# dmalyuta/explicit_hybrid_mpc

Hardware: AMD Instinct MI355X
Metric: oracle LP solves/sec + final regions/sec, 4-state 2-input N=5 hybrid MPC (higher is better)
Workload: dtype f64

## Files before the change

explicit_hybrid_mpc_amd/csrc/ehm_ipm2.h:

```cpp
#include "ehm_dev.h"

#ifndef EHM_NP
#error "EHM_NP (column capacity, multiple of 4) must be defined"
#endif
#ifndef EHM_SLOTS
#error "EHM_SLOTS (row slots per lane) must be defined"
#endif

#ifndef EHM2_UNROLL
#define EHM2_UNROLL 2
#endif
#ifndef EHM2_FORM_MFMA
#define EHM2_FORM_MFMA 0
#endif
#ifndef EHM2_LU_CHUNK
#define EHM2_LU_CHUNK 8
#endif
#define EHM2_TOL_RES      1e-10
#define EHM2_TOL_GAP      1e-10
#define EHM2_MAX_ITER     40
#define EHM2_STEP_FRAC    0.999
#define EHM2_STEP_FRAC_SAFE 0.99
#define EHM2_STEP_FRAC_LAST 0.9
#define EHM2_ATTEMPTS     3
#define EHM2_PIVOT_REL    1e-13
#define EHM2_PIVOT_BIG    1e128
#define EHM2_STALL_ZONE   1e4
#define EHM2_ACCEPT_MERIT 1e3

#define EHM2_CAT2(a, b, c) a##b##_##c
#define EHM2_CAT(a, b, c) EHM2_CAT2(a, b, c)
#ifndef EHM2_QUAD
#define EHM2_QUAD 0
#endif
#if EHM2_QUAD
#define EHM2_NS EHM2_CAT(ehm2q_, EHM_NP, EHM_SLOTS)
#else
#define EHM2_NS EHM2_CAT(ehm2_, EHM_NP, EHM_SLOTS)
#endif

#ifndef EHM2_PROF
#define EHM2_PROF 0
#endif

namespace EHM2_NS {

using namespace ehm;

#if EHM2_PROF
#define EHM2_PT(k)                                                                   \
    {                                                                                \
        const long long _t = (long long)__builtin_readcyclecounter();               \
        if (lane0 == 0) W.pf[k] += (unsigned long long)(_t - _tp);                   \
        _tp = _t;                                                                    \
    }
#define EHM2_PDUMP()                                                                 \
    {                                                                                \
        wsync();                                                                     \
        if (S.gprof && lane0 < 24)                                                   \
            atomicAdd(&S.gprof[lane0], W.pf[lane0] + (lane0 == 23 ? 1ULL : 0ULL));   \
    }
#elif defined(EHM2_ISA_MARKS)
#define EHM2_PT(k) asm volatile("; @@PHASE " #k);
#define EHM2_PDUMP()
#else
#define EHM2_PT(k)
#define EHM2_PDUMP()
#endif

constexpr int NP = EHM_NP;
constexpr int SLOTS = EHM_SLOTS;
constexpr int MROWS = 64 * SLOTS;

__device__ __forceinline__ void wsync() {
    __builtin_amdgcn_fence(__ATOMIC_ACQ_REL, "wavefront");
    __builtin_amdgcn_wave_barrier();
}

template <int CTRL, int ROW_MASK>
__device__ __forceinline__ double dpp_move(double identity, double v) {
    const int lo = __builtin_amdgcn_update_dpp(__double2loint(identity), __double2loint(v), CTRL,
                                               ROW_MASK, 0xf, false);
    const int hi = __builtin_amdgcn_update_dpp(__double2hiint(identity), __double2hiint(v), CTRL,
                                               ROW_MASK, 0xf, false);
    return __hiloint2double(hi, lo);
}
__device__ __forceinline__ double lane63(double v) {
    const int lo = __builtin_amdgcn_readlane(__double2loint(v), 63);
    const int hi = __builtin_amdgcn_readlane(__double2hiint(v), 63);
    return __hiloint2double(hi, lo);
}
#define EHM2_DPP_REDUCE(OP, IDENT)                                       \
    v = OP(v, dpp_move<0x111, 0xf>(IDENT, v));                           \
    v = OP(v, dpp_move<0x112, 0xf>(IDENT, v));                           \
    v = OP(v, dpp_move<0x114, 0xf>(IDENT, v));                           \
    v = OP(v, dpp_move<0x118, 0xf>(IDENT, v));                           \
    v = OP(v, dpp_move<0x142, 0xa>(IDENT, v));                           \
    v = OP(v, dpp_move<0x143, 0xc>(IDENT, v));                           \
    return lane63(v);
__device__ __forceinline__ double op_add(double a, double b) { return a + b; }
__device__ __forceinline__ double op_max(double a, double b) { return fmax(a, b); }
__device__ __forceinline__ double op_min(double a, double b) { return fmin(a, b); }
#ifdef EHM2_REDUCE_SHFL
__device__ __forceinline__ double wave_sum(double v) {
    for (int o = 32; o > 0; o >>= 1) v += __shfl_xor(v, o, 64);
    return v;
}
__device__ __forceinline__ double wave_max(double v) {
    for (int o = 32; o > 0; o >>= 1) v = fmax(v, __shfl_xor(v, o, 64));
    return v;
}
#else
__device__ __forceinline__ double wave_sum(double v) { EHM2_DPP_REDUCE(op_add, 0.0) }
__device__ __forceinline__ double wave_max(double v) {
    EHM2_DPP_REDUCE(op_max, -__builtin_huge_val())
}
#endif
__device__ __forceinline__ double readlane_d(double v, int src) {
    const int lo = __builtin_amdgcn_readlane(__double2loint(v), src);
    const int hi = __builtin_amdgcn_readlane(__double2hiint(v), src);
    return __hiloint2double(hi, lo);
}
__device__ __forceinline__ int pin(int x) {
    asm volatile("" : "+v"(x));
    return x;
}
typedef __attribute__((address_space(3))) const volatile double lds_cvdouble;
__device__ __forceinline__ double lds1(const double* p) {
    return *(lds_cvdouble*)p;
}
__device__ __forceinline__ double uniform_d(double v) {
    int lo, hi;
    asm("s_nop 0\n\tv_readfirstlane_b32 %0, %2\n\tv_readfirstlane_b32 %1, %3\n\ts_nop 1"
        : "=s"(lo), "=s"(hi)
        : "v"(__double2loint(v)), "v"(__double2hiint(v)));
    return __hiloint2double(hi, lo);
}
__device__ __forceinline__ double const_d(double literal) {
    int lo = __double2loint(literal), hi = __double2hiint(literal);
    asm volatile("" : "+s"(lo), "+s"(hi));
    return __hiloint2double(hi, lo);
}
__device__ __forceinline__ double frcp(double x) {
    double r = __builtin_amdgcn_rcp(x);
    double e = fma(-x, r, 1.0);
    r = fma(r, e, r);
    e = fma(-x, r, 1.0);
    r = fma(r, e, r);
    return r;
}

struct Shared {
    const double* Wc;
    const double* wv;
    const double* cv;
    const double* aE;
    const double* eval;
    const int* erow;
    const int* eidx;
    int n, m, p, lda;
    int nd0, nE, LE;
    int colS, colOne, colZero;
#if EHM2_PROF
    unsigned long long* gprof;
#endif
};
__host__ __device__ inline size_t shared_doubles(const DevProblem& P) {
    return (((size_t)P.tot4 + (P.wc_lds ? P.m + P.n : 0)) + 1) & ~(size_t)1;
}
__device__ inline void carve_shared(Shared& S, double* base, const DevProblem& P) {
    S.n = P.n; S.m = P.m; S.p = P.p; S.lda = P.lda4;
    S.nd0 = P.nd0; S.nE = P.n - P.nd0; S.LE = P.LE4;
    S.colS = P.nd0; S.colOne = P.nd0 + P.p; S.colZero = P.nd0 + P.p + 1;
#if EHM2_PROF
    S.gprof = nullptr;
#endif
    S.Wc = base;
    S.aE = base + (size_t)(P.nd0 + P.p + 2) * P.lda4;
    S.eval = base + (size_t)P.ncw4 * P.lda4;
    S.erow = reinterpret_cast<const int*>(S.eval + (size_t)S.nE * S.LE);
    S.eidx = S.erow + (size_t)S.nE * S.LE;
    if (P.wc_lds) {
        S.wv = base + P.tot4;
        S.cv = S.wv + P.m;
    } else {
        S.wv = P.w;
        S.cv = P.c;
    }
}
__device__ inline void use_commutation(Shared& S, const DevProblem& P, int d) {
    if (!P.wc_lds) S.wv = P.w + (size_t)d * P.m;
}
__device__ inline void load_shared(const DevProblem& P, int d, double* base, int tid, int nthr) {
    const int tot = P.tot4;
    const double* src = P.Wc4 + (size_t)d * tot;
    for (int k = tid; k < tot; k += nthr) base[k] = src[k];
    if (P.wc_lds) {
        const double* wd = P.w + (size_t)d * P.m;
        for (int k = tid; k < P.m; k += nthr) base[tot + k] = wd[k];
        for (int k = tid; k < P.n; k += nthr) base[tot + P.m + k] = P.c[k];
    }
}

struct Wave {
    double* M;
    double* X;
    double* vm0;
    double* vm1;
    double* c;
    double* x;
    double* xb;
    double* t;
// ... 151 lines not shown
    int lane;
};
__device__ __forceinline__ void make_rowmap(RowMap& rm, const Shared& S, const Wave& W, int lane) {
    rm.lane = lane;
    const int zero_off = S.colZero * S.lda;
#pragma unroll
    for (int sl = 0; sl < SLOTS - 1; ++sl) rm.valid[sl] = (lane + 64 * sl) < S.m;
    const int i = lane + 64 * (SLOTS - 1);
    const bool spec = W.n_lin < W.nr;
    rm.last_extra = false;
    rm.last_sx = -1;
    if (i < S.m) {
        rm.valid[SLOTS - 1] = true;
        rm.last_base = S.Wc + i;
        rm.last_stride = S.lda;
        rm.last_spec = S.Wc + (spec ? W.spec_col * S.lda : zero_off) + i;
    } else if (i >= W.xbase + W.nsx && i < W.xbase + W.ne) {
        rm.valid[SLOTS - 1] = true;
        rm.last_extra = true;
        rm.last_base = W.X + (i - W.xbase - W.nsx);
        rm.last_stride = W.ldx;
        rm.last_spec = W.X + (size_t)W.n_lin * W.ldx + (i - W.xbase - W.nsx);
    } else if (i >= W.xbase && i < W.xbase + W.nsx) {
        rm.valid[SLOTS - 1] = true;
        rm.last_sx = i - W.xbase;
        rm.last_base = S.Wc + zero_off;
        rm.last_stride = 0;
        rm.last_spec = S.Wc + zero_off;
    } else {
        rm.valid[SLOTS - 1] = false;
        rm.last_base = S.Wc + zero_off;
        rm.last_stride = 0;
        rm.last_spec = S.Wc + zero_off;
    }
}

__device__ __forceinline__ void to_psi(const Wave& W, const double* v, int lane) {
    if (lane < NP) {
        double y = (lane < W.nr) ? v[lane] : 0.0;
        const int r = lane - W.psi0;
        if (r >= 0 && r < W.npsi) {
            y = 0.0;
            for (int q = 0; q < W.npsi; ++q) y = fma(W.E[r * W.npsi + q], v[W.psi0 + q], y);
        }
        W.yv[lane] = y;
    }
    wsync();
}

__device__ __forceinline__ void rows_times(const Shared& S, const Wave& W, int lane,
                                           const double* v, double (&out)[SLOTS]) {
    RowMap rm;
    make_rowmap(rm, S, W, lane);
    to_psi(W, v, rm.lane);
    const double* y = W.yv;
#pragma unroll
    for (int sl = 0; sl < SLOTS; ++sl) out[sl] = 0.0;
    const double* pa = S.Wc + rm.lane;
    const double* pb = rm.last_base;
    const double* pv = rm.last_extra ? v : y;
    const int lda = S.lda;
    const int str = rm.last_stride;
    int j = 0;
    constexpr int UR = EHM2_UNROLL;
    for (; j + UR - 1 < W.n_lin; j += UR) {
        double a[UR][SLOTS], yj[UR], vl[UR];
#pragma unroll
        for (int u = 0; u < UR; ++u) {
            yj[u] = y[j + u];
            vl[u] = lds1(pv + j + u);
#pragma unroll
            for (int sl = 0; sl < SLOTS - 1; ++sl) a[u][sl] = lds1(pa + u * lda + 64 * sl);
            a[u][SLOTS - 1] = lds1(pb + u * str);
        }
#pragma unroll
        for (int u = 0; u < UR; ++u) {
#pragma unroll
            for (int sl = 0; sl < SLOTS - 1; ++sl) out[sl] = fma(a[u][sl], yj[u], out[sl]);
            out[SLOTS - 1] = fma(a[u][SLOTS - 1], vl[u], out[SLOTS - 1]);
        }
        pa += UR * lda;
        pb += UR * str;
    }
    for (; j < W.n_lin; ++j) {
        const double yj = y[j];
#pragma unroll
        for (int sl = 0; sl < SLOTS - 1; ++sl) out[sl] = fma(lds1(pa + 64 * sl), yj, out[sl]);
        out[SLOTS - 1] = fma(lds1(pb), lds1(pv + j), out[SLOTS - 1]);
        pa += lda;
        pb += str;
    }
    if (W.n_lin < W.nr) {
        const double vj = v[W.n_lin];
        const double* ps = S.Wc + (size_t)W.spec_col * lda + rm.lane;
#pragma unroll
        for (int sl = 0; sl < SLOTS - 1; ++sl) out[sl] = fma(ps[64 * sl], vj, out[sl]);
        out[SLOTS - 1] = fma(*rm.last_spec, vj, out[SLOTS - 1]);
    }
    if (W.nE > 0) {
        const double* vE = v + W.nr;
#pragma unroll
        for (int sl = 0; sl < SLOTS; ++sl) {
            const int i = rm.lane + 64 * sl;
            const int ic = (i < S.m) ? i : 0;
            const double a = (i < S.m) ? S.aE[ic] : 0.0;
            out[sl] = fma(a, vE[S.eidx[ic]], out[sl]);
        }
        if (rm.last_extra) {
            const int xe = rm.lane + 64 * (SLOTS - 1) - W.xbase - W.nsx;
            const double* xr = W.X + (size_t)W.nr * W.ldx + xe;
            double a = 0.0;
            for (int e = 0; e < W.nE; ++e) a = fma(xr[(size_t)e * W.ldx], vE[e], a);
            out[SLOTS - 1] += a;
        }
    }
    if (W.nsx > 0) {
        double sb = 0.0;
        for (int q = 0; q < W.npsi; ++q) sb += v[W.psi0 + q];
        if (rm.last_sx >= 0)
            out[SLOTS - 1] = (rm.last_sx < W.npsi) ? -v[W.psi0 + (rm.last_sx < W.npsi ? rm.last_sx : 0)]
                                                  : sb;
    }
#pragma unroll
    for (int sl = 0; sl < SLOTS; ++sl) out[sl] = rm.valid[sl] ? out[sl] : 0.0;
}

__device__ __forceinline__ void block_cols_mpc(const Shared& S, const Wave& W, int cb,
                                               const double* (&pc)[4]) {
    const double* zero = S.Wc + (size_t)S.colZero * S.lda;
#pragma unroll
    for (int q = 0; q < 4; ++q) {
        const int j = 4 * cb + q;
        pc[q] = (j < W.nr) ? (S.Wc + (size_t)wc_col(W, j) * S.lda) : zero;
    }
}
__device__ __forceinline__ void block_cols_ext(const Shared& S, const Wave& W, int cb,
                                               const double* (&px)[4]) {
    const double* zero = S.Wc + (size_t)S.colZero * S.lda;
#pragma unroll
    for (int q = 0; q < 4; ++q) {
        const int j = 4 * cb + q;
        px[q] = (j < W.nr && W.ldx > 0) ? (W.X + (size_t)j * W.ldx) : zero;
    }
}

template <bool TWO>
__device__ __forceinline__ void cols_times(const Shared& S, const Wave& W, const double* u0,
                                           const double* u1, double* sc, int lane, double& r0,
                                           double& r1) {
    constexpr int nb = NP / 4;
    constexpr int ks = 64 / nb;
    double ex0 = 0.0, ex1 = 0.0;
    if (lane < W.n_lp && W.ne > W.nsx) {
        const double* xl = W.X + (size_t)lane * W.ldx;
        const int xb0 = W.xbase + W.nsx;
        for (int e = 0; e < W.ne - W.nsx; ++e) {
            const double a = xl[e];
            ex0 = fma(a, u0[xb0 + e], ex0);
            if (TWO) ex1 = fma(a, u1[xb0 + e], ex1);
        }
    }
    {
        const int q = lane - W.psi0;
        if (W.nsx > 0 && q >= 0 && q < W.npsi) {
            ex0 += u0[W.xbase + W.npsi] - u0[W.xbase + q];
            if (TWO) ex1 += u1[W.xbase + W.npsi] - u1[W.xbase + q];
        }
    }
    const int ecol = lane - W.nr;
    const bool elane = W.nE > 0 && ecol >= 0 && ecol < W.nE;
    if (W.nE > 0) {
        const int eb = (elane ? ecol : 0) * S.LE;
        double s0 = 0.0, s1 = 0.0;
        for (int k = 0; k < S.LE; k += 4) {
            int i[4];
            double a[4], w0[4], w1[4];
#pragma unroll
            for (int u = 0; u < 4; ++u) {
                i[u] = S.erow[eb + k + u];
                a[u] = S.eval[eb + k + u];
            }
#pragma unroll
            for (int u = 0; u < 4; ++u) {
                w0[u] = lds1(u0 + i[u]);
                w1[u] = TWO ? lds1(u1 + i[u]) : 0.0;
            }
#pragma unroll
            for (int u = 0; u < 4; ++u) {
                s0 = fma(a[u], w0[u], s0);
                if (TWO) s1 = fma(a[u], w1[u], s1);
            }
        }
        ex0 = elane ? (ex0 + s0) : ex0;
        if (TWO) ex1 = elane ? (ex1 + s1) : ex1;
    }
    const int cb = pin(lane % nb);
    const int h = pin(lane / nb);
    const bool active = h < ks;
    double a0[4] = {0.0, 0.0, 0.0, 0.0}, a1[4] = {0.0, 0.0, 0.0, 0.0};
    if (active) {
        const double* pc[4];
// ... 239 lines not shown
        }
    }
    if (m4 < m) {
        const bool in = m4 + lk < m;
        const int ic = in ? m4 : (m - 1 - lk);
        const double d = in ? lds1(pd + ic) : 0.0;
        const double w0 = lds1(p0 + ic);
        const double a0 = w0 * d;
        c00 = __builtin_amdgcn_mfma_f64_16x16x4f64(a0, w0, c00, 0, 0, 0);
        if (two) {
            const double w1 = lds1(p1 + ic);
            const double a1 = w1 * d;
            c10 = __builtin_amdgcn_mfma_f64_16x16x4f64(a1, w0, c10, 0, 0, 0);
            c11 = __builtin_amdgcn_mfma_f64_16x16x4f64(a1, w1, c11, 0, 0, 0);
        }
    }
    for (int e0 = 0; e0 < W.nE; e0 += 4) {
        const int e = e0 + lk;
        const bool in = e < W.nE;
        const int ec = in ? e : 0;
        const double id = W.iD[ec];
        const double g0 = (in && j0 < NP) ? W.gE[ec * GS + (j0 < NP ? j0 : 0)] : 0.0;
        c00 = __builtin_amdgcn_mfma_f64_16x16x4f64(-g0 * id, g0, c00, 0, 0, 0);
        if (two) {
            const double g1 = (in && j1 < NP) ? W.gE[ec * GS + (j1 < NP ? j1 : 0)] : 0.0;
            c10 = __builtin_amdgcn_mfma_f64_16x16x4f64(-g1 * id, g0, c10, 0, 0, 0);
            c11 = __builtin_amdgcn_mfma_f64_16x16x4f64(-g1 * id, g1, c11, 0, 0, 0);
        }
    }
    wsync();
#pragma unroll
    for (int r = 0; r < 4; ++r) {
        const int row = lk + 4 * r, col = li;
        if (row < NP && col < NP) W.M[row * LDM + col] = c00[r];
        if (two) {
            if (16 + row < NP && col < NP) {
                W.M[(16 + row) * LDM + col] = c10[r];
                W.M[col * LDM + 16 + row] = c10[r];
            }
            if (16 + row < NP && 16 + col < NP) W.M[(16 + row) * LDM + 16 + col] = c11[r];
        }
    }
}

__device__ __forceinline__ void form_eliminated(const Shared& S, const Wave& W, const double* dvec,
                                                int lane) {
    constexpr int NPG = (NP > 16) ? 32 : 16;
    const double* zero = S.Wc + (size_t)S.colZero * S.lda;
    const int ntask = W.nE * NPG;
    for (int t0 = 0; t0 < ntask; t0 += 64) {
        const int t = t0 + lane;
        const int r = t & (NPG - 1);
        const int e = t / NPG;
        const bool in = t < ntask;
        const double* col = (in && r < W.n_mpc) ? (S.Wc + (size_t)wc_col(W, r) * S.lda) : zero;
        const int eb = (in ? e : 0) * S.LE;
        double g = 0.0, dl = 0.0;
        for (int k = 0; k < S.LE; k += 4) {
            int i[4];
            double ev[4], dv[4], av[4];
#pragma unroll
            for (int u = 0; u < 4; ++u) {
                i[u] = S.erow[eb + k + u];
                ev[u] = S.eval[eb + k + u];
            }
#pragma unroll
            for (int u = 0; u < 4; ++u) {
                dv[u] = lds1(dvec + i[u]);
                av[u] = lds1(col + i[u]);
            }
#pragma unroll
            for (int u = 0; u < 4; ++u) {
                const double de = dv[u] * ev[u];
                g = fma(de, av[u], g);
                dl = fma(de, ev[u], dl);
            }
        }
        if (in && r < NP) W.gE[e * GS + r] = g;
        if (in && r == 0) W.iD[e] = frcp(dl);
    }
    wsync();
}

__device__ __forceinline__ double row16_sum(double v) {
    v += dpp_move<0x111, 0xf>(0.0, v);
    v += dpp_move<0x112, 0xf>(0.0, v);
    v += dpp_move<0x114, 0xf>(0.0, v);
    v += dpp_move<0x118, 0xf>(0.0, v);
    return readlane_d(v, 15);
}
__device__ __forceinline__ double few_sum(double v, int cnt) {
    return (cnt <= 16) ? row16_sum(v) : wave_sum(v);
}

template <int P>
__device__ __forceinline__ void to_beta_form(const Wave& W, const double* dext, int lane) {
    const int p0 = W.psi0;
    const double* Em = W.E;
    double tmp[P];
    if (lane < NP) {
        double* mr = W.M + lane * LDM + p0;
        double v[P];
#pragma unroll
        for (int r = 0; r < P; ++r) v[r] = mr[r];
#pragma unroll
        for (int q = 0; q < P; ++q) {
            double a = 0.0;
#pragma unroll
            for (int r = 0; r < P; ++r) a = fma(v[r], Em[r * P + q], a);
            tmp[q] = a;
        }
#pragma unroll
        for (int q = 0; q < P; ++q) mr[q] = tmp[q];
    }
    for (int e = lane; e < W.nE; e += 64) {
        double* gr = W.gE + e * GS + p0;
        double v[P];
#pragma unroll
        for (int r = 0; r < P; ++r) v[r] = gr[r];
#pragma unroll
        for (int q = 0; q < P; ++q) {
            double a = 0.0;
#pragma unroll
            for (int r = 0; r < P; ++r) a = fma(v[r], Em[r * P + q], a);
            gr[q] = a;
        }
    }
    wsync();
    if (lane < NP) {
        double* mc = W.M + p0 * LDM + lane;
        double v[P];
#pragma unroll
        for (int r = 0; r < P; ++r) v[r] = mc[r * LDM];
#pragma unroll
        for (int q = 0; q < P; ++q) {
            double a = 0.0;
#pragma unroll
            for (int r = 0; r < P; ++r) a = fma(Em[r * P + q], v[r], a);
            tmp[q] = a;
        }
#pragma unroll
        for (int q = 0; q < P; ++q) mc[q * LDM] = tmp[q];
    }
    wsync();
    if (lane < P) {
        const double dsum = dext[P];
        double* mr = W.M + (p0 + lane) * LDM + p0;
#pragma unroll
        for (int q = 0; q < P; ++q) mr[q] += dsum + ((q == lane) ? dext[lane] : 0.0);
    }
    wsync();
}

__device__ __forceinline__ void form_normal_matrix(const Shared& S, const Wave& W, const double* dvec,
                                          const double* dext, int lane
#if EHM2_PROF
                                          , int lane0, long long& _tp
#endif
                                          ) {
    if (W.nE > 0) form_eliminated(S, W, dvec, lane);
    EHM2_PT(2)
    int nbA;
    if (EHM2_FORM_MFMA || W.n_mpc <= 16) {
        nbA = (W.n_mpc > 16 || NP <= 16) ? (NP >> 2) : 4;
        form_mfma(S, W, dvec, lane, W.n_mpc);
    } else {
        nbA = (W.n_mpc + 3) >> 2;
        const int TA = nbA * (nbA + 1) / 2;
        const int ks = 64 / TA;
        if (ks >= 8) form_blocks_ks<8>(S, W, dvec, lane, nbA, TA);
        else if (NP >= 16 && ks >= 6) form_blocks_ks<6>(S, W, dvec, lane, nbA, TA);
        else if (NP >= 20 && ks >= 4) form_blocks_ks<4>(S, W, dvec, lane, nbA, TA);
        else if (NP >= 24 && ks == 3) form_blocks_ks<3>(S, W, dvec, lane, nbA, TA);
        else if (NP >= 28 && ks == 2) form_blocks_ks<2>(S, W, dvec, lane, nbA, TA);
        else if (NP >= 32) form_blocks<1, 1>(S, W, dvec, lane, nbA, TA);
// ... 33 lines not shown
        const bool bad = !(piv > const_d(EHM2_PIVOT_REL) * orig) || !(piv > 0.0);
        piv = bad ? const_d(EHM2_PIVOT_BIG) : piv;
        const double rinv = frcp(piv);
        if (lane == 0) W.db[k] = rinv;
        const double l = row[k] * rinv;
        row[k] = l;
        if (((k + 1) & 1) && k + 1 < NP) {
            const double ukq = U[uoff(k) + k + 1];
            row[k + 1] = fma(-l, ukq, row[k + 1]);
        }
#pragma unroll
        for (int q = (k + 2) & ~1; q < NP; q += 2) {
            const double2v u = *reinterpret_cast<const double2v*>(U + uoff(k) + q);
            row[q] = fma(-l, u.x, row[q]);
            row[q + 1] = fma(-l, u.y, row[q + 1]);
            if (((q - ((k + 2) & ~1)) / 2) % (EHM2_LU_CHUNK / 2) == EHM2_LU_CHUNK / 2 - 1)
                __builtin_amdgcn_sched_barrier(0);
        }
#pragma unroll
        for (int q = k + 1; q < NP; ++q) asm volatile("" : "+v"(row[q]));
    }
    wsync();
}

__device__ __forceinline__ void masked_fnma(double& bv, double a, double s, unsigned long long mask) {
    unsigned long long sv;
    asm volatile("s_and_saveexec_b64 %[sv], %[m]\n\t"
                 "v_fma_f64 %[bv], -%[a], %[s], %[bv]\n\t"
                 "s_mov_b64 exec, %[sv]\n\t"
                 "s_nop 0"
                 : [bv] "+v"(bv), [sv] "=&s"(sv)
                 : [a] "v"(a), [s] "s"(s), [m] "s"(mask)
                 : "scc");
}

__device__ __forceinline__ double lu_solve(const double (&row)[NP], const Wave& W, double rinv,
                                           double rhs, int lane) {
    double bv = rhs;
#pragma unroll
    for (int k = 0; k < NP - 1; ++k) {
        const double yk = readlane_d(bv, k);
        bv = fma(-row[k], yk, bv);
    }
    const int jl = (lane < NP) ? lane : (NP - 1);
    const double* urow = W.M + uoff(jl);
#pragma unroll
    for (int k = NP - 1; k >= 1; --k) {
        const double xk = readlane_d(bv * rinv, k);
        masked_fnma(bv, urow[k], xk, (1ull << k) - 1ull);
    }
    const double x = bv * rinv;
    if (lane < W.nr) W.t[lane] = x;
    wsync();
    return x;
}

__device__ __forceinline__ void dense_prep(const Shared& S, const Wave& W, const double* dext,
                                           int lane) {
    const int kd = W.ne - W.nsx;
    if (kd <= 0) return;
    const int e0 = W.nsx;
    const int nEp = (W.nE + 1) & ~1;
    const bool two = kd > 1;
    double g11 = frcp(dext[e0]);
    double g22 = two ? frcp(dext[e0 + 1]) : 1.0;
    double g12 = 0.0;
    double x0 = 0.0, x1 = 0.0;
    if (lane < W.nr) {
        x0 = W.X[(size_t)lane * W.ldx];
        x1 = two ? W.X[(size_t)lane * W.ldx + 1] : 0.0;
    }
    if (W.nE > 0) {
        const bool el = lane < W.nE;
        const double* xr = W.X + (size_t)(W.nr + (el ? lane : 0)) * W.ldx;
        const double xe0 = el ? xr[0] : 0.0;
        const double xe1 = (el && two) ? xr[1] : 0.0;
        const double id = el ? W.iD[el ? lane : 0] : 0.0;
        const double h0 = xe0 * id, h1 = xe1 * id;
        if (el) {
            W.hX[lane] = h0;
            W.hX[nEp + lane] = h1;
        }
        wsync();
        if (lane < W.nr)
            for (int e = 0; e < W.nE; ++e) {
                const double g = W.gE[e * GS + lane];
                x0 = fma(-W.hX[e], g, x0);
                x1 = fma(-W.hX[nEp + e], g, x1);
            }
        g11 += few_sum(h0 * xe0, W.nE);
        if (two) {
            g12 = few_sum(h0 * xe1, W.nE);
            g22 += few_sum(h1 * xe1, W.nE);
        }
    }
    const double i1 = frcp(g11);
    const double l = g12 * i1;
    const double i2 = two ? frcp(fma(-l, g12, g22)) : 0.0;
    x1 = fma(-l, x0, x1);
    if (lane < NP) {
        W.xh[lane] = x0;
        W.xh[NP + lane] = two ? x1 : 0.0;
    }
    if (lane == 0) {
        W.dn[0] = l;
        W.dn[1] = i1;
        W.dn[2] = i2;
    }
    wsync();
}

__device__ __forceinline__ double solve_full(const double (&row)[NP], const Shared& S,
                                             const Wave& W, double rinv, double rhs, int lane) {
    const int kd = W.ne - W.nsx;
    const bool two = kd > 1;
    const int e = lane - W.nr;
    const bool el = W.nE > 0 && e >= 0 && e < W.nE;
    const int jl = (lane < NP) ? lane : (NP - 1);
    double rho0 = 0.0, rho1 = 0.0;
    double rr = (lane < W.nr) ? rhs : 0.0;
    if (W.nE > 0) {
        if (el) W.qE[e] = rhs * W.iD[e];
        wsync();
        if (lane < W.nr)
            for (int e2 = 0; e2 < W.nE; ++e2) rr = fma(-W.gE[e2 * GS + lane], W.qE[e2], rr);
        if (kd > 0) {
            const bool l2 = lane < W.nE;
            const double* xr = W.X + (size_t)(W.nr + (l2 ? lane : 0)) * W.ldx;
            const double q = l2 ? W.qE[l2 ? lane : 0] : 0.0;
            rho0 = few_sum(l2 ? xr[0] * q : 0.0, W.nE);
            if (two) rho1 = few_sum(l2 ? xr[1] * q : 0.0, W.nE);
        }
    }
    double l = 0.0, i1 = 0.0, i2 = 0.0;
    if (kd > 0) {
        l = W.dn[0];
        i1 = W.dn[1];
        i2 = W.dn[2];
        rho1 = fma(-l, rho0, rho1);
        rr = fma(-W.xh[jl], i1 * rho0, rr);
        rr = fma(-W.xh[NP + jl], i2 * rho1, rr);
    }
    const double xD = lu_solve(row, W, rinv, rr, lane);
    double y0 = 0.0, y1 = 0.0;
    if (kd > 0 && W.nE > 0) {
        const bool lr = lane < W.nr;
        const double v0 = few_sum(lr ? W.xh[jl] * xD : 0.0, W.nr) + rho0;
        const double v1 = two ? (few_sum(lr ? W.xh[NP + jl] * xD : 0.0, W.nr) + rho1) : 0.0;
        y1 = v1 * i2;
        y0 = fma(-l, y1, v0 * i1);
    }
    if (W.nE > 0) {
        double xE = 0.0;
        if (el) {
            double acc = rhs;
            const double* ge = W.gE + e * GS;
            for (int j = 0; j < W.nr; ++j) acc = fma(-ge[j], W.t[j], acc);
            if (kd > 0) {
                const double* xr = W.X + (size_t)(W.nr + e) * W.ldx;
                acc = fma(-xr[0], y0, acc);
                if (two) acc = fma(-xr[1], y1, acc);
            }
            xE = acc * W.iD[e];
            W.t[W.nr + e] = xE;
        }
        wsync();
        return el ? xE : xD;
    }
    return xD;
}

__device__ __forceinline__ IpmResult ipm_solve(const Shared& S, const Wave& W, const double (&b)[SLOTS],
                                      int lane0, int sign_only, double step_frac,
                                      double* gout = nullptr) {
    int lane = lane0;
    const int n = W.n_lp;
    const int m_lp = S.m + W.ne;
    RowMap rm;
    make_rowmap(rm, S, W, lane);
    double s[SLOTS], lam[SLOTS], v[SLOTS];
    double bmax = 0.0;
#pragma unroll
    for (int sl = 0; sl < SLOTS; ++sl) {
        v[sl] = rm.valid[sl] ? b[sl] : 0.0;
        s[sl] = rm.valid[sl] ? fmax(b[sl], 1.0) : 1.0;
        lam[sl] = rm.valid[sl] ? 1.0 : 0.0;
        bmax = fmax(bmax, fabs(v[sl]));
    }
    const double bnorm = uniform_d(1.0 + wave_max(bmax));
    const double cj = (lane < n) ? W.c[lane] : 0.0;
    const double cnorm = uniform_d(1.0 + wave_max(fabs(cj)));
    step_frac = uniform_d(step_frac);
    if (lane < n) {
        W.x[lane] = 0.0;
        W.xb[lane] = 0.0;
    }
#pragma unroll
    for (int sl = 0; sl < SLOTS; ++sl) {
        if (!rm.valid[sl]) {
            W.vm0[lane + 64 * sl] = 0.0;
            W.vm1[lane + 64 * sl] = 0.0;
        }
    }
    wsync();

#if EHM2_PROF
    if (lane0 < 24) W.pf[lane0] = 0ULL;
    wsync();
    long long _tp = (long long)__builtin_readcyclecounter();
#endif
    IpmResult res;
    res.obj = 0.0;
    res.merit = const_d(1e300);
    res.iters = 0;
    res.status = 1;
    int stall = 0;
    int m_op = __builtin_amdgcn_readfirstlane(m_lp);
    asm volatile("" : "+s"(m_op));
    const double inv_m = uniform_d(frcp((double)m_op));

    for (int it = 0; it <= EHM2_MAX_ITER; ++it) {
        lane = pin(lane0);
#if EHM2_QUAD
        double xQx = 0.0, qx = 0.0, gjj = 0.0;
        if (W.quad) {
            const double xj = (lane < n) ? W.x[lane] : 0.0;
            const double qj = (lane < n) ? W.qv[lane] : 0.0;
            double g = 0.0;
            if (lane < n) {
                const double* qrow = W.Q + lane * LDM;
                for (int k = 0; k < n; ++k) g = fma(qrow[k], W.x[k], g);
            }
            xQx = wave_sum(xj * g);
            qx = wave_sum(xj * qj);
            const double gvj = g + qj;
            gjj = (lane < n) ? W.kap0 * gvj : 0.0;
            if (W.eq >= 0) {
                const double a1j = (lane < n) ? W.a1[lane] : 0.0;
                const double a2j = (lane < n) ? W.a2[lane] : 0.0;
                if (lane < n) {
                    W.X[(size_t)lane * W.ldx + W.eq - W.nsx] = fma(W.kap1, gvj, a1j);
                    W.X[(size_t)lane * W.ldx + W.eq - W.nsx + 1] = fma(W.kap2, gvj, a2j);
                }
                const double a1x = wave_sum(a1j * xj);
                const double a2x = wave_sum(a2j * xj);
                const int e = lane + 64 * (SLOTS - 1) - W.xbase;
                const double Vx = fma(0.5, xQx, qx);
                if (rm.last_extra && e == W.eq) v[SLOTS - 1] = W.bq1 - fma(W.kap1, Vx, a1x);
                if (rm.last_extra && e == W.eq + 1) v[SLOTS - 1] = W.bq2 - fma(W.kap2, Vx, a2x);
            }
            wsync();
        }
#endif
        double r_p[SLOTS], rs[SLOTS];
        double rpmax = 0.0, sl_sum = 0.0, vl_sum = 0.0;
#pragma unroll
        for (int sl = 0; sl < SLOTS; ++sl) {
            r_p[sl] = rm.valid[sl] ? (s[sl] - v[sl]) : 0.0;
            rpmax = fmax(rpmax, fabs(r_p[sl]));
            sl_sum = fma(s[sl], lam[sl], sl_sum);
            vl_sum = fma(v[sl], lam[sl], vl_sum);
            rs[sl] = frcp(s[sl]);
        }
#pragma unroll
        for (int sl = 0; sl < SLOTS; ++sl) {
            if (rm.valid[sl]) {
                W.vm0[lane + 64 * sl] = lam[sl];
                W.vm1[lane + 64 * sl] = lam[sl] * rs[sl] * r_p[sl];
            }
        }
        wsync();
        EHM2_PT(0)
        double atl, atdr;
        cols_times<true>(S, W, W.vm0, W.vm1, W.M, lane, atl, atdr);
        EHM2_PT(1)
        const double cjj = (lane < n) ? W.c[lane] : 0.0;
        const double xjj = (lane < n) ? W.x[lane] : 0.0;
#if EHM2_QUAD
        const double r_d = (lane < n) ? (atl + cjj + gjj) *
            (W.quad ? rsqrt(1.0 + W.Q[lane * LDM + lane]) : 1.0) : 0.0;
        const double cn = W.quad ? (1.0 + wave_max(fmax(fabs(cjj), fabs(gjj)))) : cnorm;
        const double emax = wave_max(fmax(rpmax / bnorm, fabs(r_d) / cn));
        const double sl_tot = wave_sum(sl_sum);
        const double mu = sl_tot * inv_m;
        double pobj = wave_sum(cjj * xjj);
        double dobj = -wave_sum(vl_sum + xjj * atl);
        if (W.quad) {
            pobj += W.kap0 * (fma(0.5, xQx, qx) + W.v0);
            dobj = pobj - sl_tot;
        }
        const double e_g = fabs(pobj - dobj) / (1.0 + fabs(pobj));
#else
        const double r_d = (lane < n) ? (atl + cjj) : 0.0;
        const double emax = wave_max(fmax(rpmax / bnorm, fabs(r_d) / cnorm));
        const double mu = wave_sum(sl_sum) * inv_m;
        const double dobj = -wave_sum(vl_sum + xjj * atl);
        const double pobj = wave_sum(cjj * xjj);
        const double e_g = fabs(pobj - dobj) / (1.0 + fabs(pobj));
#endif
        const double merit = fmax(emax / const_d(EHM2_TOL_RES), e_g / const_d(EHM2_TOL_GAP));
        if (!(mu == mu) || !(pobj == pobj) || fabs(pobj) > const_d(1e300)) {
            res.merit = const_d(1e300);
            res.obj = pobj;
            res.status = 1;
            res.iters = it;
            break;
        }
        if (merit < res.merit) {
            res.merit = uniform_d(merit);
            res.obj = uniform_d(pobj);
            stall = 0;
            if (lane < n) W.xb[lane] = W.x[lane];
        } else if (res.merit < const_d(EHM2_STALL_ZONE)) {
            ++stall;
        }
        res.iters = it;
        if (merit <= 1.0) {
            res.status = 0;
            break;
        }
        if (sign_only && emax <= const_d(EHM2_SIGN_RES) && pobj * dobj > 0.0 &&
            (sign_only == 1 || pobj > 0.0)) {
            const double lo = fmin(fabs(pobj), fabs(dobj));
            if (lo >= W.sign_floor && fabs(pobj - dobj) <= const_d(EHM2_SIGN_GAP) * lo &&
                emax * (1.0 + fabs(pobj)) <= const_d(EHM2_SIGN_RES_REL) * lo) {
                res.obj = pobj;
                res.merit = merit;
                res.margin = lo;
                res.status = 0;
                if (lane < n) W.xb[lane] = W.x[lane];
                wsync();
                EHM2_PT(15)
                EHM2_PDUMP()
                return res;
            }
        }
        if (stall >= 3 || it == EHM2_MAX_ITER || !(merit == merit)) break;

        EHM2_PT(15)
        lane = pin(lane0);
#pragma unroll
        for (int sl = 0; sl < SLOTS; ++sl)
            if (rm.valid[sl]) W.vm0[lane + 64 * sl] = lam[sl] * rs[sl];
        wsync();
        if (rm.last_extra || rm.last_sx >= 0)
            W.ub[lane + 64 * (SLOTS - 1) - W.xbase] = lam[SLOTS - 1] * rs[SLOTS - 1];
#if EHM2_QUAD
        if (W.quad && W.eq >= 0 && rm.last_extra) {
            const int e = lane + 64 * (SLOTS - 1) - W.xbase;
            if (e == W.eq) W.lq[0] = lam[SLOTS - 1];
            if (e == W.eq + 1) W.lq[1] = lam[SLOTS - 1];
        }
#endif
        wsync();
#if EHM2_PROF
        form_normal_matrix(S, W, W.vm0, W.ub, lane, lane0, _tp);
#else
        form_normal_matrix(S, W, W.vm0, W.ub, lane);
#endif
        EHM2_PT(4)
        lane = pin(lane0);
        dense_prep(S, W, W.ub, lane);
        EHM2_PT(5)
        lane = pin(lane0);
        double row[NP];
        {
            const int jr = (lane < NP) ? lane : (NP - 1);
            const double* mrow = W.M + jr * LDM;
#pragma unroll
            for (int q = 0; q < NP; ++q) row[q] = mrow[q];
            double dg = mrow[jr];
            for (int r = 0; r < W.ne - W.nsx; ++r) {
                const double* xh = W.xh + r * NP;
                const double xl = xh[jr];
                const double ce = W.dn[1 + r] * xl;
                dg = fma(ce, xl, dg);
#pragma unroll
                for (int q = 0; q < NP; ++q) {
                    row[q] = fma(ce, xh[q], row[q]);
                    if ((q & 3) == 3) __builtin_amdgcn_sched_barrier(0);
                }
            }
#if EHM2_QUAD
            if (W.quad) {
                double wq = W.kap0;
                if (W.eq >= 0) wq = fma(W.kap1, W.lq[0], fma(W.kap2, W.lq[1], wq));
                const int jl = (lane < NP) ? lane : (NP - 1);
                const double* qrow = W.Q + jl * LDM;
                const bool in = jl < W.n_lp;
#pragma unroll
                for (int q = 0; q < NP; ++q)
                    row[q] = fma(wq, (in && q < W.n_lp) ? qrow[q] : 0.0, row[q]);
                dg = fma(wq, in ? qrow[jl] : 0.0, dg);
            }
#endif
            if (lane < NP) W.db[lane] = dg;
        }
        wsync();
        EHM2_PT(6)
        lu_factor(row, W, lane);
#pragma unroll
        for (int k = 0; k < NP; ++k) row[k] = (k < lane) ? row[k] : 0.0;
        EHM2_PT(7)
        const double rinv_l = W.db[(lane < NP) ? lane : (NP - 1)];

        lane = pin(lane0);
#if EHM2_QUAD
        const double rhs_aff = (lane < n) ? (-cjj - gjj - atdr) : 0.0;
#else
        const double rhs_aff = (lane < n) ? (-cjj - atdr) : 0.0;
#endif
        double dxj = solve_full(row, S, W, rinv_l, rhs_aff, lane);
        EHM2_PT(8)
        double adx[SLOTS];
        rows_times(S, W, lane, W.t, adx);
        EHM2_PT(9)
        double ds_a[SLOTS], dl_a[SLOTS];
        double rho_p = 0.0, rho_d = 0.0;
#pragma unroll
        for (int sl = 0; sl < SLOTS; ++sl) {
            ds_a[sl] = rm.valid[sl] ? (-r_p[sl] - adx[sl]) : 0.0;
            dl_a[sl] = rm.valid[sl] ? (-lam[sl] - lam[sl] * rs[sl] * ds_a[sl]) : 0.0;
            rho_p = fmax(rho_p, -ds_a[sl] * rs[sl]);
            rho_d = fmax(rho_d, rm.valid[sl] ? fma(ds_a[sl], rs[sl], 1.0) : 0.0);
        }
        rho_p = wave_max(rho_p);
        rho_d = wave_max(rho_d);
        double ap = (rho_p > 1.0) ? 1.0 / rho_p : 1.0;
        double ad = (rho_d > 1.0) ? 1.0 / rho_d : 1.0;
#if EHM2_QUAD
        if (W.quad) ap = ad = fmin(ap, ad);
#endif
        double mu_aff = 0.0;
#pragma unroll
        for (int sl = 0; sl < SLOTS; ++sl)
            if (rm.valid[sl])
                mu_aff = fma(s[sl] + ap * ds_a[sl], lam[sl] + ad * dl_a[sl], mu_aff);
        mu_aff = wave_sum(mu_aff) * inv_m;
        const double ratio = mu_aff / mu;
        const double sigma = ratio * ratio * ratio;
        const double smu = sigma * mu;

        lane = pin(lane0);
#pragma unroll
        for (int sl = 0; sl < SLOTS; ++sl) {
            if (rm.valid[sl]) W.vm1[lane + 64 * sl] = (ds_a[sl] * dl_a[sl] - smu) * rs[sl];
        }
        wsync();
        double atc, dummy;
        EHM2_PT(10)
        cols_times<false>(S, W, W.vm1, W.vm1, W.sc, lane, atc, dummy);
        EHM2_PT(11)
        const double rhs = (lane < n) ? (rhs_aff + atc) : 0.0;
        dxj = solve_full(row, S, W, rinv_l, rhs, lane);
        EHM2_PT(12)
        rows_times(S, W, lane, W.t, adx);
        EHM2_PT(13)
        double ds[SLOTS], dl[SLOTS];
        rho_p = 0.0;
        rho_d = 0.0;
#pragma unroll
        for (int sl = 0; sl < SLOTS; ++sl) {
            const double corr = rm.valid[sl] ? W.vm1[lane + 64 * sl] : 0.0;
            const double rl = frcp(rm.valid[sl] ? lam[sl] : 1.0);
            ds[sl] = rm.valid[sl] ? (-r_p[sl] - adx[sl]) : 0.0;
            dl[sl] = rm.valid[sl] ? (-lam[sl] - corr - lam[sl] * rs[sl] * ds[sl]) : 0.0;
            rho_p = fmax(rho_p, -ds[sl] * rs[sl]);
            rho_d = fmax(rho_d, -dl[sl] * rl);
        }
        rho_p = wave_max(rho_p);
        rho_d = wave_max(rho_d);
        ap = (rho_p > step_frac) ? step_frac / rho_p : 1.0;
        ad = (rho_d > step_frac) ? step_frac / rho_d : 1.0;
#if EHM2_QUAD
        if (W.quad) ap = ad = fmin(ap, ad);
#endif
        if (lane < n) W.x[lane] = fma(ap, dxj, W.x[lane]);
#pragma unroll
        for (int sl = 0; sl < SLOTS; ++sl) {
            if (rm.valid[sl]) {
                s[sl] = fma(ap, ds[sl], s[sl]);
                lam[sl] = fma(ad, dl[sl], lam[sl]);
                v[sl] = fma(-ap, adx[sl], v[sl]);
            }
        }
        wsync();
        EHM2_PT(14)
    }
    wsync();
    EHM2_PDUMP()
    if (gout) {
        const bool conv = (res.status == 0) && (res.merit <= 1.0);
        for (int q = 0; q < S.p; ++q) {
            const double* col = S.Wc + (size_t)(S.colS + q) * S.lda + lane0;
            double a = 0.0;
#pragma unroll
            for (int sl = 0; sl < SLOTS; ++sl)
                if (lane0 + 64 * sl < S.m) a = fma(col[64 * sl], lam[sl], a);
            a = wave_sum(a);
            if (lane0 == 0) gout[q] = conv ? a : __builtin_nan("");
        }
        wsync();
    }
    if (res.status != 0 && res.merit <= const_d(EHM2_ACCEPT_MERIT)) res.status = 0;
    res.margin = fabs(res.obj);
    return res;
}

}
```

Measured before the change: 10.40 million.

## Batch wave reductions and unroll LDS dot-product loops in IPM kernel

Adds batched DPP wave reductions that process several values per stage, using bound_ctrl zero-fill for non-negative max and sum so no identity register copies are needed. Independent reductions in the IPM iteration (mu/dobj/pobj sums, rho_p/rho_d maxes, few_sum triples) are merged so their DPP latencies interleave. Scalar LDS dot-product and sum loops (extra rows, psi sums, gE/hX updates, qE back-substitution) are unrolled with pinned volatile LDS pointers to issue loads ahead of the FMAs. The zero-fill max variant assumes the reduced values are non-negative, and the extra unrolled code may raise register pressure.

```diff
diff --git a/explicit_hybrid_mpc_amd/csrc/ehm_ipm2.h b/explicit_hybrid_mpc_amd/csrc/ehm_ipm2.h
--- a/explicit_hybrid_mpc_amd/csrc/ehm_ipm2.h
+++ b/explicit_hybrid_mpc_amd/csrc/ehm_ipm2.h
@@ -83,6 +83,19 @@
                                                ROW_MASK, 0xf, false);
     const int hi = __builtin_amdgcn_update_dpp(__double2hiint(identity), __double2hiint(v), CTRL,
                                                ROW_MASK, 0xf, false);
+    return __hiloint2double(hi, lo);
+}
+__device__ __forceinline__ int any_vgpr() {
+    int x;
+    asm volatile("" : "=v"(x));
+    return x;
+}
+template <int CTRL, int ROW_MASK>
+__device__ __forceinline__ double dpp_fill0(double v) {
+    const int olo = (ROW_MASK == 0xf) ? 0 : any_vgpr();
+    const int ohi = (ROW_MASK == 0xf) ? 0 : any_vgpr();
+    const int lo = __builtin_amdgcn_update_dpp(olo, __double2loint(v), CTRL, ROW_MASK, 0xf, true);
+    const int hi = __builtin_amdgcn_update_dpp(ohi, __double2hiint(v), CTRL, ROW_MASK, 0xf, true);
     return __hiloint2double(hi, lo);
 }
 __device__ __forceinline__ double lane63(double v) {
@@ -110,8 +123,43 @@
     for (int o = 32; o > 0; o >>= 1) v = fmax(v, __shfl_xor(v, o, 64));
     return v;
 }
+__device__ __forceinline__ double wave_max_nn(double v) { return wave_max(v); }
+template <int N>
+__device__ __forceinline__ void wave_sums(double (&v)[N]) {
+#pragma unroll
+    for (int i = 0; i < N; ++i) v[i] = wave_sum(v[i]);
+}
+template <int N>
+__device__ __forceinline__ void wave_maxs_nn(double (&v)[N]) {
+#pragma unroll
+    for (int i = 0; i < N; ++i) v[i] = wave_max(v[i]);
+}
 #else
-__device__ __forceinline__ double wave_sum(double v) { EHM2_DPP_REDUCE(op_add, 0.0) }
+#define EHM2_DPP_STAGE(OP, CTRL, ROW_MASK)                                                 \
+    _Pragma("unroll") for (int i = 0; i < N; ++i)                                          \
+        v[i] = OP(v[i], dpp_fill0<CTRL, ROW_MASK>(v[i]));
+#define EHM2_DPP_REDUCE_FILL0(OP)                                        \
+    EHM2_DPP_STAGE(OP, 0x111, 0xf)                                       \
+    EHM2_DPP_STAGE(OP, 0x112, 0xf)                                       \
+    EHM2_DPP_STAGE(OP, 0x114, 0xf)                                       \
+    EHM2_DPP_STAGE(OP, 0x118, 0xf)                                       \
+    EHM2_DPP_STAGE(OP, 0x142, 0xa)                                       \
+    EHM2_DPP_STAGE(OP, 0x143, 0xc)                                       \
+    _Pragma("unroll") for (int i = 0; i < N; ++i) v[i] = lane63(v[i]);
+template <int N>
+__device__ __forceinline__ void wave_sums(double (&v)[N]) { EHM2_DPP_REDUCE_FILL0(op_add) }
+template <int N>
+__device__ __forceinline__ void wave_maxs_nn(double (&v)[N]) { EHM2_DPP_REDUCE_FILL0(op_max) }
+__device__ __forceinline__ double wave_sum(double x) {
+    double v[1] = {x};
+    wave_sums(v);
+    return v[0];
+}
+__device__ __forceinline__ double wave_max_nn(double x) {
+    double v[1] = {x};
+    wave_maxs_nn(v);
+    return v[0];
+}
 __device__ __forceinline__ double wave_max(double v) {
     EHM2_DPP_REDUCE(op_max, -__builtin_huge_val())
 }
@@ -128,6 +176,55 @@
 typedef __attribute__((address_space(3))) const volatile double lds_cvdouble;
 __device__ __forceinline__ double lds1(const double* p) {
     return *(lds_cvdouble*)p;
+}
+typedef __attribute__((address_space(3))) const volatile double* lds_vptr;
+__device__ __forceinline__ lds_vptr lds_pin(const double* p) {
+    lds_vptr q = (lds_vptr)p;
+    asm volatile("" : "+v"(q));
+    return q;
+}
+template <int B, bool NEG>
+__device__ __forceinline__ double fma_run(const double* a_, int sa, const double* b_, int sb,
+                                          int cnt, double acc) {
+    lds_vptr a = lds_pin(a_), b = lds_pin(b_);
+    int r = cnt;
+    for (; r >= B; r -= B) {
+        double av[B], bv[B];
+#pragma unroll
+        for (int u = 0; u < B; ++u) {
+            av[u] = *a;
+            bv[u] = *b;
+            a += sa;
+            b += sb;
+        }
+#pragma unroll
+        for (int u = 0; u < B; ++u) acc = fma(NEG ? -av[u] : av[u], bv[u], acc);
+    }
+    for (; r > 0; --r) {
+        const double av = *a;
+        acc = fma(NEG ? -av : av, *b, acc);
+        a += sa;
+        b += sb;
+    }
+    return acc;
+}
+template <int B>
+__device__ __forceinline__ double add_run(const double* a_, int cnt, double acc) {
+    lds_vptr a = lds_pin(a_);
+    int r = cnt;
+    for (; r >= B; r -= B) {
+        double av[B];
+#pragma unroll
+        for (int u = 0; u < B; ++u) av[u] = a[u];
+#pragma unroll
+        for (int u = 0; u < B; ++u) acc += av[u];
+        a += B;
+    }
+    for (; r > 0; --r) {
+        acc += *a;
+        ++a;
+    }
+    return acc;
 }
 __device__ __forceinline__ double uniform_d(double v) {
     int lo, hi;
@@ -445,13 +542,26 @@
         pa += UR * lda;
         pb += UR * str;
     }
-    for (; j < W.n_lin; ++j) {
-        const double yj = y[j];
-#pragma unroll
-        for (int sl = 0; sl < SLOTS - 1; ++sl) out[sl] = fma(lds1(pa + 64 * sl), yj, out[sl]);
-        out[SLOTS - 1] = fma(lds1(pb), lds1(pv + j), out[SLOTS - 1]);
-        pa += lda;
-        pb += str;
+    if (j < W.n_lin) {
+        constexpr int UL = (UR > 1) ? UR - 1 : 1;
+        double a[UL][SLOTS], yj[UL], vl[UL];
+        const int left = W.n_lin - j;
+#pragma unroll
+        for (int u = 0; u < UL; ++u)
+            if (u < left) {
+                yj[u] = y[j + u];
+                vl[u] = lds1(pv + j + u);
+#pragma unroll
+                for (int sl = 0; sl < SLOTS - 1; ++sl) a[u][sl] = lds1(pa + u * lda + 64 * sl);
+                a[u][SLOTS - 1] = lds1(pb + u * str);
+            }
+#pragma unroll
+        for (int u = 0; u < UL; ++u)
+            if (u < left) {
+#pragma unroll
+                for (int sl = 0; sl < SLOTS - 1; ++sl) out[sl] = fma(a[u][sl], yj[u], out[sl]);
+                out[SLOTS - 1] = fma(a[u][SLOTS - 1], vl[u], out[SLOTS - 1]);
+            }
     }
     if (W.n_lin < W.nr) {
         const double vj = v[W.n_lin];
@@ -472,14 +582,11 @@
         if (rm.last_extra) {
             const int xe = rm.lane + 64 * (SLOTS - 1) - W.xbase - W.nsx;
             const double* xr = W.X + (size_t)W.nr * W.ldx + xe;
-            double a = 0.0;
-            for (int e = 0; e < W.nE; ++e) a = fma(xr[(size_t)e * W.ldx], vE[e], a);
-            out[SLOTS - 1] += a;
+            out[SLOTS - 1] += fma_run<4, false>(xr, pin(W.ldx), vE, 1, W.nE, 0.0);
         }
     }
     if (W.nsx > 0) {
-        double sb = 0.0;
-        for (int q = 0; q < W.npsi; ++q) sb += v[W.psi0 + q];
+        const double sb = add_run<4>(v + W.psi0, W.npsi, 0.0);
         if (rm.last_sx >= 0)
             out[SLOTS - 1] = (rm.last_sx < W.npsi) ? -v[W.psi0 + (rm.last_sx < W.npsi ? rm.last_sx : 0)]
                                                   : sb;
@@ -885,15 +992,34 @@
     wsync();
 }
 
-__device__ __forceinline__ double row16_sum(double v) {
-    v += dpp_move<0x111, 0xf>(0.0, v);
-    v += dpp_move<0x112, 0xf>(0.0, v);
-    v += dpp_move<0x114, 0xf>(0.0, v);
-    v += dpp_move<0x118, 0xf>(0.0, v);
-    return readlane_d(v, 15);
-}
-__device__ __forceinline__ double few_sum(double v, int cnt) {
-    return (cnt <= 16) ? row16_sum(v) : wave_sum(v);
+template <int N>
+__device__ __forceinline__ void row16_sums(double (&v)[N]) {
+#ifdef EHM2_REDUCE_SHFL
+#pragma unroll
+    for (int i = 0; i < N; ++i) {
+        v[i] += dpp_move<0x111, 0xf>(0.0, v[i]);
+        v[i] += dpp_move<0x112, 0xf>(0.0, v[i]);
+        v[i] += dpp_move<0x114, 0xf>(0.0, v[i]);
+        v[i] += dpp_move<0x118, 0xf>(0.0, v[i]);
+    }
+#else
+    EHM2_DPP_STAGE(op_add, 0x111, 0xf)
+    EHM2_DPP_STAGE(op_add, 0x112, 0xf)
+    EHM2_DPP_STAGE(op_add, 0x114, 0xf)
+    EHM2_DPP_STAGE(op_add, 0x118, 0xf)
+#endif
+#pragma unroll
+    for (int i = 0; i < N; ++i) v[i] = readlane_d(v[i], 15);
+}
+template <int N>
+__device__ __forceinline__ void few_sums(double (&v)[N], int cnt) {
+    if (cnt <= 16) row16_sums(v);
+    else wave_sums(v);
+}
+__device__ __forceinline__ double few_sum(double x, int cnt) {
+    double v[1] = {x};
+    few_sums(v, cnt);
+    return v[0];
 }
 
 template <int P>
@@ -1093,16 +1219,41 @@
             W.hX[nEp + lane] = h1;
         }
         wsync();
-        if (lane < W.nr)
-            for (int e = 0; e < W.nE; ++e) {
-                const double g = W.gE[e * GS + lane];
-                x0 = fma(-W.hX[e], g, x0);
-                x1 = fma(-W.hX[nEp + e], g, x1);
-            }
-        g11 += few_sum(h0 * xe0, W.nE);
+        if (lane < W.nr) {
+            lds_vptr pg = lds_pin(W.gE + lane), ph = lds_pin(W.hX);
+            int left = W.nE;
+            for (; left >= 5; left -= 5) {
+                double g[5], a0[5], a1[5];
+#pragma unroll
+                for (int u = 0; u < 5; ++u) {
+                    g[u] = pg[u * GS];
+                    a0[u] = ph[u];
+                    a1[u] = ph[nEp + u];
+                }
+#pragma unroll
+                for (int u = 0; u < 5; ++u) {
+                    x0 = fma(-a0[u], g[u], x0);
+                    x1 = fma(-a1[u], g[u], x1);
+                }
+                pg += 5 * GS;
+                ph += 5;
+            }
+            for (; left > 0; --left) {
+                const double g = *pg;
+                x0 = fma(-*ph, g, x0);
+                x1 = fma(-ph[nEp], g, x1);
+                pg += GS;
+                ++ph;
+            }
+        }
         if (two) {
-            g12 = few_sum(h0 * xe1, W.nE);
-            g22 += few_sum(h1 * xe1, W.nE);
+            double gs[3] = {h0 * xe0, h0 * xe1, h1 * xe1};
+            few_sums(gs, W.nE);
+            g11 += gs[0];
+            g12 = gs[1];
+            g22 += gs[2];
+        } else {
+            g11 += few_sum(h0 * xe0, W.nE);
         }
     }
     const double i1 = frcp(g11);
@@ -1133,14 +1284,19 @@
     if (W.nE > 0) {
         if (el) W.qE[e] = rhs * W.iD[e];
         wsync();
-        if (lane < W.nr)
-            for (int e2 = 0; e2 < W.nE; ++e2) rr = fma(-W.gE[e2 * GS + lane], W.qE[e2], rr);
+        if (lane < W.nr) rr = fma_run<5, true>(W.gE + lane, GS, W.qE, 1, W.nE, rr);
         if (kd > 0) {
             const bool l2 = lane < W.nE;
             const double* xr = W.X + (size_t)(W.nr + (l2 ? lane : 0)) * W.ldx;
             const double q = l2 ? W.qE[l2 ? lane : 0] : 0.0;
-            rho0 = few_sum(l2 ? xr[0] * q : 0.0, W.nE);
-            if (two) rho1 = few_sum(l2 ? xr[1] * q : 0.0, W.nE);
+            if (two) {
+                double rs2[2] = {l2 ? xr[0] * q : 0.0, l2 ? xr[1] * q : 0.0};
+                few_sums(rs2, W.nE);
+                rho0 = rs2[0];
+                rho1 = rs2[1];
+            } else {
+                rho0 = few_sum(l2 ? xr[0] * q : 0.0, W.nE);
+            }
         }
     }
     double l = 0.0, i1 = 0.0, i2 = 0.0;
@@ -1156,8 +1312,15 @@
     double y0 = 0.0, y1 = 0.0;
     if (kd > 0 && W.nE > 0) {
         const bool lr = lane < W.nr;
-        const double v0 = few_sum(lr ? W.xh[jl] * xD : 0.0, W.nr) + rho0;
-        const double v1 = two ? (few_sum(lr ? W.xh[NP + jl] * xD : 0.0, W.nr) + rho1) : 0.0;
+        double v0, v1 = 0.0;
+        if (two) {
+            double vs[2] = {lr ? W.xh[jl] * xD : 0.0, lr ? W.xh[NP + jl] * xD : 0.0};
+            few_sums(vs, W.nr);
+            v0 = vs[0] + rho0;
+            v1 = vs[1] + rho1;
+        } else {
+            v0 = few_sum(lr ? W.xh[jl] * xD : 0.0, W.nr) + rho0;
+        }
         y1 = v1 * i2;
         y0 = fma(-l, y1, v0 * i1);
     }
@@ -1198,9 +1361,9 @@
         lam[sl] = rm.valid[sl] ? 1.0 : 0.0;
         bmax = fmax(bmax, fabs(v[sl]));
     }
-    const double bnorm = uniform_d(1.0 + wave_max(bmax));
+    const double bnorm = uniform_d(1.0 + wave_max_nn(bmax));
     const double cj = (lane < n) ? W.c[lane] : 0.0;
-    const double cnorm = uniform_d(1.0 + wave_max(fabs(cj)));
+    const double cnorm = uniform_d(1.0 + wave_max_nn(fabs(cj)));
     step_frac = uniform_d(step_frac);
     if (lane < n) {
         W.x[lane] = 0.0;
@@ -1290,8 +1453,8 @@
 #if EHM2_QUAD
         const double r_d = (lane < n) ? (atl + cjj + gjj) *
             (W.quad ? rsqrt(1.0 + W.Q[lane * LDM + lane]) : 1.0) : 0.0;
-        const double cn = W.quad ? (1.0 + wave_max(fmax(fabs(cjj), fabs(gjj)))) : cnorm;
-        const double emax = wave_max(fmax(rpmax / bnorm, fabs(r_d) / cn));
+        const double cn = W.quad ? (1.0 + wave_max_nn(fmax(fabs(cjj), fabs(gjj)))) : cnorm;
+        const double emax = wave_max_nn(fmax(rpmax / bnorm, fabs(r_d) / cn));
         const double sl_tot = wave_sum(sl_sum);
         const double mu = sl_tot * inv_m;
         double pobj = wave_sum(cjj * xjj);
@@ -1303,10 +1466,12 @@
         const double e_g = fabs(pobj - dobj) / (1.0 + fabs(pobj));
 #else
         const double r_d = (lane < n) ? (atl + cjj) : 0.0;
-        const double emax = wave_max(fmax(rpmax / bnorm, fabs(r_d) / cnorm));
-        const double mu = wave_sum(sl_sum) * inv_m;
-        const double dobj = -wave_sum(vl_sum + xjj * atl);
-        const double pobj = wave_sum(cjj * xjj);
+        const double emax = wave_max_nn(fmax(rpmax / bnorm, fabs(r_d) / cnorm));
+        double sums[3] = {sl_sum, vl_sum + xjj * atl, cjj * xjj};
+        wave_sums(sums);
+        const double mu = sums[0] * inv_m;
+        const double dobj = -sums[1];
+        const double pobj = sums[2];
         const double e_g = fabs(pobj - dobj) / (1.0 + fabs(pobj));
 #endif
         const double merit = fmax(emax / const_d(EHM2_TOL_RES), e_g / const_d(EHM2_TOL_GAP));
@@ -1435,8 +1600,12 @@
             rho_p = fmax(rho_p, -ds_a[sl] * rs[sl]);
             rho_d = fmax(rho_d, rm.valid[sl] ? fma(ds_a[sl], rs[sl], 1.0) : 0.0);
         }
-        rho_p = wave_max(rho_p);
-        rho_d = wave_max(rho_d);
+        {
+            double rho[2] = {rho_p, rho_d};
+            wave_maxs_nn(rho);
+            rho_p = rho[0];
+            rho_d = rho[1];
+        }
         double ap = (rho_p > 1.0) ? 1.0 / rho_p : 1.0;
         double ad = (rho_d > 1.0) ? 1.0 / rho_d : 1.0;
 #if EHM2_QUAD
@@ -1479,8 +1648,12 @@
             rho_p = fmax(rho_p, -ds[sl] * rs[sl]);
             rho_d = fmax(rho_d, -dl[sl] * rl);
         }
-        rho_p = wave_max(rho_p);
-        rho_d = wave_max(rho_d);
+        {
+            double rho[2] = {rho_p, rho_d};
+            wave_maxs_nn(rho);
+            rho_p = rho[0];
+            rho_d = rho[1];
+        }
         ap = (rho_p > step_frac) ? step_frac / rho_p : 1.0;
         ad = (rho_d > step_frac) ? step_frac / rho_d : 1.0;
 #if EHM2_QUAD
```

Result: faster. 10.86 million (median of 6 runs) (+4.4%).
